# Zaggy1024/RaytracerCore

Hardware: AMD Instinct MI355X
Metric: Mrays/sec (primary+secondary) and samples/sec at 1080p, Cornell box (higher is better)
Workload: dtype f32; 1 GPU; bounce.txt camera 0 1920x1080 x 256 spp per GPU per step; traversal=brute, recursion=10, kernel_build=scene-specialised (hiprtc)

## Files before the change

### include/rtcore.h

```cpp
#ifndef RTCORE_H
#define RTCORE_H

#ifndef __HIPCC_RTC__
#include <stdint.h>
#include <stddef.h>
#endif

#ifdef __cplusplus
extern "C" {
#endif

#define RTCORE_ABI_VERSION 6

typedef enum rt_status {
    RT_OK = 0,
    RT_ERR_ARG = -1,
    RT_ERR_HIP = -2,
    RT_ERR_OOM = -3,
    RT_ERR_NCCL = -4,
    RT_ERR_PARSE = -5,
    RT_ERR_NODEVICE = -6,
    RT_ERR_STATE = -7
} rt_status;

// ... 79 lines not shown
    RT_BVH_BUILDER_GPU = 2
} rt_bvh_builder;

#define RT_BUILD_STATS_COUNT 22

int rt_abi_version(void);
const char* rt_build_info(void);
int rt_device_count(void);
int rt_last_error(char* buf, int32_t cap);

int rt_scene_create(const rt_scene_params* params, const rt_prim* prims, int32_t n_prims,
                    int32_t device, rt_scene** out_scene);
int rt_scene_set_camera(rt_scene* scene, const rt_camera* camera);
int rt_scene_set_traversal(rt_scene* scene, int32_t traversal);
int rt_scene_get_info(const rt_scene* scene, rt_scene_info* info);
void rt_scene_destroy(rt_scene* scene);
int rt_set_bvh_builder(int32_t builder);
int rt_scene_get_build_stats(const rt_scene* scene, double* out, int32_t n);
int rt_set_jit(int32_t on);
int rt_scene_get_jit_error(const rt_scene* scene, char* buf, int32_t cap);
int rt_debug_jit_compile(const char* arch, int32_t grouped, char* log, int32_t cap);
int rt_debug_jit_header(const rt_scene_params* params, const rt_prim* prims, int32_t n_prims, const rt_camera* camera,
                        int32_t grouped, char* buf, int64_t cap);
int rt_scene_check_bvh(rt_scene* scene);
#define RT_LAYOUT_COUNT 10
int rt_debug_brute_layout(const rt_prim* prims, int32_t n_prims, int32_t* out, int32_t n_out);
int rt_debug_item_order(int32_t w, int32_t h, int32_t spp, int32_t chunks, int32_t pool, int32_t band,
                        int32_t band_stride, int32_t band_offset, uint32_t* out, int64_t cap_words, int32_t* info);
int rt_debug_pixels_plan(int32_t kernel, int64_t n, int32_t spp, int32_t* info);
int rt_debug_scene_bound(const rt_prim* prims, int32_t n_prims, float* lo, float* hi, float* info);
int rt_debug_block_cull(const rt_prim* prims, int32_t n_prims, const rt_camera* camera, int32_t width, int32_t height,
                        int32_t x0, int32_t y0, int32_t w, int32_t h, int32_t band, int32_t band_stride,
                        int32_t band_offset, uint8_t* dead, int64_t cap, int32_t* info);
int rt_debug_ray_log(rt_scene* scene, void* d_log, uint32_t cap, void* d_count);
int rt_debug_vn_rehit(const double* v0, const double* e01, const double* e02, int32_t mirror, double u, double v,
                      const float* dir, int32_t* inside, double* t, double* origin);
int rt_debug_trace_rays(rt_scene* scene, const void* d_rays, uint32_t n, void* d_hits, int32_t waves_per_simd,
                        void* d_stats, void* stream, float* ms);

int rt_render_tile(rt_scene* scene, int32_t x0, int32_t y0, int32_t w, int32_t h, int32_t spp,
                   uint64_t seed, uint64_t sample_base, rt_color* sum_rgb, uint32_t* samples,
                   uint32_t* misses, uint64_t* rays_out);

int rt_render_tile_1spp(rt_scene* scene, int32_t x0, int32_t y0, int32_t w, int32_t h,
                        uint64_t seed, uint64_t sample_index, rt_color* out);

int rt_primary_ids(rt_scene* scene, int32_t x0, int32_t y0, int32_t w, int32_t h, int32_t* ids_out);

int rt_bvh_counts(rt_scene* scene, int32_t x0, int32_t y0, int32_t w, int32_t h, int32_t* counts_out);

typedef enum rt_bounce_type {
    RT_BOUNCE_SKIPPED = 0,
    RT_BOUNCE_DIFFUSE = 1,
    RT_BOUNCE_SPECULAR = 2,
    RT_BOUNCE_SPECULAR_FAIL = 3,
    RT_BOUNCE_TRANSMITTED = 4,
    RT_BOUNCE_EMISSION = 5,
    RT_BOUNCE_PURE_BLACK = 6,
    RT_BOUNCE_RECURSION_COMPLETE = 7,
    RT_BOUNCE_MISSED = 8,
    RT_BOUNCE_DEBUG = 9
} rt_bounce_type;

typedef struct rt_debug_ray {
    int32_t prim_id;
    int32_t type;
// ... 167 lines not shown
```

### raytracercore_amd/__init__.py

```python
from __future__ import annotations

import ctypes as C
import enum
import os
from dataclasses import dataclass
from typing import List, Optional, Sequence, Tuple

import numpy as np

_HERE = os.path.dirname(os.path.abspath(__file__))
LIB_PATH = os.path.join(_HERE, "librtcore_hip.so")
REPO_ROOT = os.path.dirname(_HERE)

RT_OK = 0
ABI_VERSION = 6
RT_PRIM_TRIANGLE, RT_PRIM_SPHERE, RT_PRIM_PLANE = 0, 1, 2
RT_FLAG_MIRROR, RT_FLAG_TWOSIDED, RT_FLAG_INVERT, RT_FLAG_HASNORMALS, RT_FLAG_TRANSFORMED = 1, 2, 4, 8, 16
RT_CAMERA_FRUSTUM, RT_CAMERA_ORTHO = 0, 1
RT_TRAVERSAL_AUTO, RT_TRAVERSAL_BRUTE, RT_TRAVERSAL_BVH, RT_TRAVERSAL_BVH2, RT_TRAVERSAL_GROUPED = 0, 1, 2, 3, 4
RT_BVH_BUILDER_AUTO, RT_BVH_BUILDER_HOST, RT_BVH_BUILDER_GPU = 0, 1, 2
(RT_BOUNCE_SKIPPED, RT_BOUNCE_DIFFUSE, RT_BOUNCE_SPECULAR, RT_BOUNCE_SPECULAR_FAIL, RT_BOUNCE_TRANSMITTED,
 RT_BOUNCE_EMISSION, RT_BOUNCE_PURE_BLACK, RT_BOUNCE_RECURSION_COMPLETE, RT_BOUNCE_MISSED, RT_BOUNCE_DEBUG) = range(10)
BOUNCE_TYPE_NAMES = ("Skipped", "Diffuse", "Specular", "SpecularFail", "Transmitted", "Emission", "PureBlack",
                     "RecursionComplete", "Missed", "Debug")
# ... 202 lines not shown
        "rt_scene_set_stats": (C.c_int, [C.c_void_p, C.c_int32]),
        "rt_scene_get_stats": (C.c_int, [C.c_void_p, P(C.c_uint64), C.c_int32]),
        "rt_render_frame_multi": (C.c_int, [P(rt_scene_params), P(rt_prim), C.c_int32, P(rt_camera), C.c_int32,
                                            C.c_int32, C.c_uint64, C.c_uint64, P(rt_color), P(C.c_uint32),
                                            P(C.c_uint32), P(C.c_uint64)]),
        "rt_render_bands": (C.c_int, [C.c_void_p] + [C.c_int32] * 4 + [C.c_uint64, C.c_uint64, P(rt_color),
                                      P(C.c_uint32), P(C.c_uint32), P(C.c_uint64)]),
        "rt_render_bands_device": (C.c_int, [C.c_void_p] + [C.c_int32] * 4 + [C.c_uint64, C.c_uint64] +
                                   [C.c_void_p] * 3 + [C.c_uint64, C.c_void_p, C.c_void_p]),
        "rt_band_rows": (C.c_int, [C.c_int32] * 4),
        "rt_band_slot_rows": (C.c_int, [C.c_int32] * 3),
        "rt_scatter_band_slot": (C.c_int, [C.c_void_p, C.c_uint64] + [C.c_int32] * 5 + [P(rt_color), P(C.c_uint32),
                                                                                       P(C.c_uint32)]),
        "rt_frame_create": (C.c_int, [P(rt_scene_params), P(rt_prim), C.c_int32, P(rt_camera), C.c_int32,
                                      P(C.c_void_p)]),
        "rt_frame_set_camera": (C.c_int, [C.c_void_p, P(rt_camera)]),
        "rt_frame_render": (C.c_int, [C.c_void_p, C.c_int32, C.c_uint64, C.c_uint64, P(rt_color), P(C.c_uint32),
                                      P(C.c_uint32), P(C.c_uint64)]),
        "rt_frame_submit": (C.c_int, [C.c_void_p, C.c_int32, C.c_uint64, C.c_uint64]),
        "rt_frame_collect": (C.c_int, [C.c_void_p, P(rt_color), P(C.c_uint32), P(C.c_uint32), P(C.c_uint64)]),
        "rt_frame_inject_fault": (C.c_int, [C.c_void_p, C.c_int32]),
        "rt_frame_destroy": (None, [C.c_void_p]),
        "rt_parse_scene": (C.c_int, [C.c_char_p, P(rt_scene_params), P(rt_prim), P(C.c_int32), P(rt_camera),
                                     P(C.c_int32)]),
        "rt_sample_output": (C.c_int32, [rt_color, C.c_uint32, C.c_uint32, rt_color, C.c_double, C.c_double]),
        "rt_tonemap_device": (C.c_int, [C.c_void_p, C.c_void_p, C.c_void_p, C.c_int32, C.c_int32, rt_color, C.c_double,
                                        C.c_double, C.c_void_p, C.c_void_p]),
        "rt_ref_bvh_export": (C.c_int, [P(rt_prim), C.c_int32, P(C.c_int32), P(C.c_double), P(C.c_int32),
                                        P(C.c_int32)]),
        "rt_debug_item_order": (C.c_int, [C.c_int32] * 8 + [P(C.c_uint32), C.c_int64, P(C.c_int32)]),
        "rt_debug_scene_bound": (C.c_int, [P(rt_prim), C.c_int32, P(C.c_float), P(C.c_float), P(C.c_float)]),
        "rt_debug_block_cull": (C.c_int, [P(rt_prim), C.c_int32, P(rt_camera)] + [C.c_int32] * 9 +
                                [P(C.c_uint8), C.c_int64, P(C.c_int32)]),
        "rt_debug_ray_log": (C.c_int, [C.c_void_p, C.c_void_p, C.c_uint32, C.c_void_p]),
        "rt_debug_vn_rehit": (C.c_int, [P(C.c_double), P(C.c_double), P(C.c_double), C.c_int32, C.c_double,
                                        C.c_double, P(C.c_float), P(C.c_int32), P(C.c_double), P(C.c_double)]),
        "rt_debug_trace_rays": (C.c_int, [C.c_void_p, C.c_void_p, C.c_uint32, C.c_void_p, C.c_int32, C.c_void_p,
                                          C.c_void_p, P(C.c_float)]),
        "rt_query_rays": (C.c_int, [C.c_void_p, C.c_int32, C.c_void_p, C.c_int64, C.c_void_p]),
        "rt_query_rays_device": (C.c_int, [C.c_void_p, C.c_int32, C.c_void_p, C.c_int64, C.c_void_p, C.c_void_p]),
        "rt_camera_rays": (C.c_int, [P(rt_camera)] + [C.c_int32] * 6 + [C.c_void_p]),
        "rt_select_pixels": (C.c_int, [C.c_void_p, C.c_void_p] + [C.c_int32] * 5 + [C.c_void_p]),
        "rt_select_pixels_device": (C.c_int, [C.c_void_p, C.c_void_p] + [C.c_int32] * 5 + [C.c_void_p, C.c_void_p]),
        "rt_select_rays": (C.c_int, [C.c_void_p, C.c_void_p, C.c_int32, C.c_void_p, C.c_int64, C.c_void_p]),
        "rt_select_rays_device": (C.c_int, [C.c_void_p, C.c_void_p, C.c_int32, C.c_void_p, C.c_int64, C.c_void_p,
                                            C.c_void_p]),
        "rt_debug_select_rays": (C.c_int, [P(rt_prim), C.c_int32, C.c_void_p, C.c_int32, C.c_void_p, C.c_int64,
                                           C.c_void_p]),
        "rt_render_rays": (C.c_int, [C.c_void_p, C.c_void_p, C.c_int64, C.c_int32, C.c_uint64, C.c_uint64, C.c_uint64,
                                     P(rt_color), P(C.c_uint32), P(C.c_uint32), P(C.c_uint64)]),
        "rt_render_rays_device": (C.c_int, [C.c_void_p, C.c_void_p, C.c_int64, C.c_int32, C.c_uint64, C.c_uint64,
                                            C.c_uint64] + [C.c_void_p] * 4 + [C.c_void_p]),
        "rt_occluded_rays": (C.c_int, [C.c_void_p, C.c_int32, C.c_void_p, C.c_void_p, C.c_int64, C.c_void_p]),
        "rt_occluded_rays_device": (C.c_int, [C.c_void_p, C.c_int32, C.c_void_p, C.c_void_p, C.c_int64, C.c_void_p,
                                              C.c_void_p]),
        "rt_render_pixels": (C.c_int, [C.c_void_p, C.c_void_p, C.c_int64, C.c_int32, C.c_uint64, C.c_uint64,
                                       P(rt_color), P(C.c_uint32), P(C.c_uint32), P(C.c_double), P(C.c_uint32),
                                       P(C.c_uint64)]),
        "rt_render_pixels_device": (C.c_int, [C.c_void_p, C.c_void_p, C.c_int64, C.c_int32, C.c_uint64, C.c_uint64] +
                                    [C.c_void_p] * 5 + [C.c_uint64, C.c_void_p, C.c_void_p]),
        "rt_adaptive_select_device": (C.c_int, [P(rt_adaptive_params)] + [C.c_void_p] * 5 + [C.c_uint64, C.c_int32,
                                                C.c_int32, C.c_void_p, C.c_uint32, C.c_void_p, C.c_void_p]),
        "rt_debug_adaptive_select": (C.c_int64, [P(rt_adaptive_params)] + [C.c_void_p] * 5 + [C.c_uint64, C.c_int32,
                                                 C.c_int32, C.c_void_p, C.c_uint32]),
        "rt_debug_pixels_plan": (C.c_int, [C.c_int32, C.c_int64, C.c_int32, P(C.c_int32)]),
        "rt_primary_hits_device": (C.c_int, [C.c_void_p] + [C.c_int32] * 4 + [C.c_void_p, C.c_void_p]),
# ... 102 lines not shown
def scene_bound(prims: Sequence[rt_prim]) -> dict:
    lib = load_library()
    n = len(prims)
    arr = (rt_prim * max(1, n))(*prims)
    lo, hi, info = (C.c_float * 3)(), (C.c_float * 3)(), (C.c_float * 2)()
    state = lib.rt_debug_scene_bound(arr, n, lo, hi, info)
    if state < 0:
        _check(state)
    return {"lo": np.array(lo, np.float32), "hi": np.array(hi, np.float32), "limit": np.float32(info[0]),
            "pad": np.float32(info[1]), "state": int(state)}


def block_cull(prims: Sequence[rt_prim], camera: rt_camera, size: Tuple[int, int],
               window: Optional[Tuple[int, int, int, int]] = None,
               bands: Optional[Tuple[int, int, int]] = None) -> Tuple[np.ndarray, int]:
    lib = load_library()
    n = len(prims)
    arr = (rt_prim * max(1, n))(*prims)
    cam = rt_camera.from_buffer_copy(camera)
    b = bands or (0, 0, 0)
    W, H = size
    rows = lib.rt_band_rows(H, b[0], b[1], b[2]) if bands else H
    x0, y0, w, h = window or (0, 0, W, rows)
    bx, by = (w + 7) // 8, (h + 7) // 8
    dead = np.zeros(max(1, bx * by), np.uint8)
    info = (C.c_int32 * 2)()
    live = lib.rt_debug_block_cull(arr, n, C.byref(cam), W, H, x0, y0, w, h, b[0], b[1], b[2],
                                   dead.ctypes.data_as(C.POINTER(C.c_uint8)), bx * by, info)
    if live < 0:
        _check(live)
    return dead[:bx * by].reshape(by, bx).astype(bool), int(live)


def ref_bvh_export(prims: Sequence[rt_prim]) -> Tuple[np.ndarray, np.ndarray, int, int]:
    lib = load_library()
    n = len(prims)
    arr = (rt_prim * max(1, n))(*prims)
    order = np.zeros(max(1, n), np.int32)
    boxes = np.zeros((max(1, 2 * n), 8), np.float64)
    nodes, depth = C.c_int32(0), C.c_int32(0)
    _check(lib.rt_ref_bvh_export(arr, n, order.ctypes.data_as(C.POINTER(C.c_int32)),
                                 boxes.ctypes.data_as(C.POINTER(C.c_double)), C.byref(nodes), C.byref(depth)))
    return order[:n], boxes[:nodes.value], nodes.value, depth.value


def sample_output(sum_rgb: Tuple[float, float, float], samples: int, misses: int,
                  background=(0.0, 0.0, 0.0), background_alpha: float = 0.0, exposure: float = 1.0) -> int:
    lib = load_library()
    return lib.rt_sample_output(rt_color(*sum_rgb), samples, misses, rt_color(*background), background_alpha, exposure)


def device_count() -> int:
    return load_library().rt_device_count()


def camera_rays(camera: rt_camera, size: Tuple[int, int], x0: int = 0, y0: int = 0, w: Optional[int] = None,
                h: Optional[int] = None) -> np.ndarray:
    lib = load_library()
    if not hasattr(lib, "rt_camera_rays"):
        raise RtError("this build of the library has no rt_camera_rays")
    W, H = int(size[0]), int(size[1])
    w = W - x0 if w is None else w
    h = H - y0 if h is None else h
    out = np.zeros((max(w, 0), max(h, 0)), RAY_DTYPE)
    cam = rt_camera.from_buffer_copy(camera)
    _check(lib.rt_camera_rays(C.byref(cam), W, H, x0, y0, w, h, out.ctypes.data_as(C.c_void_p)))
# ... 627 lines not shown
```

### raytracercore_amd/csrc/api_debug.hip

```cpp
#include <cstdlib>
#include <cstring>

#include "rt_scene.h"

namespace {

int n_bvh_prims(const std::vector<HostPrim>& H)
{
    int nb = 0;
    for (const HostPrim& p : H) nb += p.kind != RT_PRIM_PLANE;
    return nb;
}

HostRecords report_records(const std::vector<HostPrim>& H)
{
    const bool host_tree = builder_for(n_bvh_prims(H)) == RT_BVH_BUILDER_HOST;
    return make_host_records(H, host_tree ? grouping_max_leaf(GroupingTree::LayoutReport, (int)H.size(), false) : 0,
                             group_max_default());
}

}

extern "C" {

// ... 453 lines not shown
                        int32_t band_offset, uint8_t* dead, int64_t cap, int32_t* info)
{
    const bool banded = band > 0;
    if (n_prims < 0 || (n_prims > 0 && !prims) || !camera || width <= 0 || height <= 0 || w <= 0 || h <= 0 || x0 < 0 ||
        y0 < 0 || x0 + w > width || cap < 0 || (cap > 0 && !dead) || band < 0 ||
        (camera->kind != RT_CAMERA_FRUSTUM && camera->kind != RT_CAMERA_ORTHO) ||
        (banded && (band_stride <= 0 || band_offset < 0 || band_offset >= band_stride)) || (!banded && y0 + h > height)) {
        set_error("rt_debug_block_cull: bad argument");
        return RT_ERR_ARG;
    }
    int n_planes = 0;
    for (int i = 0; i < n_prims; i++) {
        if (prims[i].kind < 0 || prims[i].kind > 2) {
            set_error("rt_debug_block_cull: unknown primitive kind at index " + std::to_string(i));
            return RT_ERR_ARG;
        }
        n_planes += prims[i].kind == RT_PRIM_PLANE ? 1 : 0;
    }
    const SceneBound b = make_scene_bound(prepare_prims(prims, n_prims));
    CameraD camd;
    CameraF camf;
    camera_init(*camera, width, height, camd, camf);
    const CullWindow win{x0, y0, w, h, banded ? band : 0, banded ? band_stride : 0, banded ? band_offset : 0};
    std::vector<unsigned char> flags;
    const int live = cull_blocks(camf, b, n_planes, win, flags);
    for (size_t i = 0; i < flags.size() && (int64_t)i < cap; i++) dead[i] = flags[i];
    if (info) {
        info[0] = (w + 7) / 8;
        info[1] = (h + 7) / 8;
    }
    return live;
}

int rt_parse_scene(const char* text, rt_scene_params* params, rt_prim* prims, int32_t* n_prims, rt_camera* cameras,
                   int32_t* n_cameras)
{
    if (!text || !n_prims || !n_cameras) {
        set_error("rt_parse_scene: bad argument");
        return RT_ERR_ARG;
    }
    ParsedScene ps;
    std::string err;
    if (!parse_scene_text(text, ps, err)) {
        set_error(err);
        return RT_ERR_PARSE;
    }
    const int cap_p = *n_prims, cap_c = *n_cameras;
    *n_prims = (int32_t)ps.prims.size();
    *n_cameras = (int32_t)ps.cameras.size();
    if (params) *params = ps.params;
    if (prims) {
        if (cap_p < (int)ps.prims.size()) {
            set_error("rt_parse_scene: primitive array too small");
            return RT_ERR_ARG;
        }
        std::copy(ps.prims.begin(), ps.prims.end(), prims);
    }
    if (cameras) {
        if (cap_c < (int)ps.cameras.size()) {
            set_error("rt_parse_scene: camera array too small");
            return RT_ERR_ARG;
        }
        std::copy(ps.cameras.begin(), ps.cameras.end(), cameras);
    }
    return RT_OK;
}
// ... 27 lines not shown
```

### raytracercore_amd/csrc/kernels_path.hip

```cpp
#include "../../include/rtcore_rng.h"
#include "rt_kernels.h"
#ifdef RT_SCENE_CONST
#include "rt_scene_const.h"
#endif

namespace rtc {
namespace {

struct V3 {
    float x, y, z;
};
__device__ __forceinline__ V3 v3(float x, float y, float z) { return V3{x, y, z}; }
__device__ __forceinline__ V3 xyz(float4 a) { return V3{a.x, a.y, a.z}; }
__device__ __forceinline__ V3 operator+(V3 a, V3 b) { return {a.x + b.x, a.y + b.y, a.z + b.z}; }
__device__ __forceinline__ V3 operator-(V3 a, V3 b) { return {a.x - b.x, a.y - b.y, a.z - b.z}; }
__device__ __forceinline__ V3 operator*(V3 a, float s) { return {a.x * s, a.y * s, a.z * s}; }
__device__ __forceinline__ V3 operator*(V3 a, V3 b) { return {a.x * b.x, a.y * b.y, a.z * b.z}; }
__device__ __forceinline__ V3 operator-(V3 a) { return {-a.x, -a.y, -a.z}; }
__device__ __forceinline__ float dot(V3 a, V3 b) { return fmaf(a.x, b.x, fmaf(a.y, b.y, a.z * b.z)); }
__device__ __forceinline__ bool known_zero(float c)
{
#if defined(RT_SCENE_CONST)
    return __builtin_constant_p(c) && c == 0.0f;
#else
// ... 609 lines not shown
    (void)c;
    return RT_SCENE_CAMERA_KIND == RT_CAMERA_FRUSTUM;
#else
    return c.kind == RT_CAMERA_FRUSTUM;
#endif
}
template <class CamT>
__device__ __forceinline__ bool cam_dof(const CamT& c)
{
#ifdef RT_SCENE_CAMERA_DOF
    (void)c;
    return RT_SCENE_CAMERA_DOF != 0;
#else
    return c.dof != 0.0f;
#endif
}
template <class CamT>
__device__ __forceinline__ Ray3 camera_ray(const CamT& c, float x, float y)
{
    Ray3 r;
    if (cam_frustum(c)) {
        const float ox = fmaf(x, c.tan_x_per_px, -c.tan_x);
        const float oy = fmaf(y, c.tan_y_per_px, -c.tan_y);
        r.d = normalize(madd(xyz(c.up), oy, madd(xyz(c.side), ox, xyz(c.look))));
        r.o = xyz(c.position);
    } else {
        r.o = madd(xyz(c.up), (y - c.h2) * c.v_mult, madd(xyz(c.side), (x - c.w2) * c.h_mult, xyz(c.position)));
        r.d = normalize(xyz(c.look));
    }
    r.o = madd(r.d, c.image_plane, r.o);
    return r;
}

template <bool LEAN = false, class CamT>
__device__ __forceinline__ void start_sample(const CamT& cam, int x, int y, Sample& S)
{
    const float sx = LEAN ? fmaf((float)rt_rng_next24(&S.rng), 0x1p-24f, (float)x) : (float)x + next_u(S.rng);
    const float sy = LEAN ? fmaf((float)rt_rng_next24(&S.rng), 0x1p-24f, (float)y) : (float)y + next_u(S.rng);
    const Ray3 r = camera_ray(cam, sx, sy);
    S.o = r.o;
    S.d = r.d;
    if (cam_dof(cam)) {
        const V3 focus = madd(r.d, cam.focal_length - cam.image_plane, r.o);
        const float dist = fsqrt(next_u(S.rng)) * cam.dof;
        const float turn = next_u(S.rng);
        const float ox = __builtin_amdgcn_cosf(turn) * dist, oy = __builtin_amdgcn_sinf(turn) * dist;
        const Ray3 r2 = camera_ray(cam, sx + ox, sy + oy);
        S.o = r2.o;
        S.d = normalize(focus - r2.o);
    }
    S.tint = v3(1.0f, 1.0f, 1.0f);
    S.bounce = 0;
    S.prev = -1;
}

template <bool LEAN>
__device__ __forceinline__ float one_minus_exp2_2a(float a, float z)
{
    const float x = 2.0f * a * 0.69314718055994531f;
    const float series = -x * fmaf(x, fmaf(x, fmaf(x, 1.0f / 24.0f, 1.0f / 6.0f), 0.5f), 1.0f);
    const float direct = LEAN ? fmaf(-z, z, 1.0f) : 1.0f - __builtin_amdgcn_exp2f(2.0f * a);
    return x > -0.0625f ? series : direct;
}

__host__ __device__ __noinline__ bool vn_rehit_test(const PrimD& P, double u, double v, V3 dir, bool& inside,
                                                   double* t_out = nullptr, double* o_out = nullptr)
{
    const Vec4d a = P.a, e1 = P.b, e2 = P.c;
    const double d[4] = {(double)dir.x, (double)dir.y, (double)dir.z, 0.0};
    const double o[4] = {__builtin_fma(e1.x, u, __builtin_fma(e2.x, v, a.x)), __builtin_fma(e1.y, u, __builtin_fma(e2.y, v, a.y)),
                         __builtin_fma(e1.z, u, __builtin_fma(e2.z, v, a.z)), __builtin_fma(e1.w, u, __builtin_fma(e2.w, v, a.w))};
// ... 342 lines not shown
    QueryRay q;
    q.o = v3((float)r0.x, (float)r0.y, (float)r1.x);
    q.d = v3((float)r2.x, (float)r2.y, (float)r3.x);
    const float inf = __builtin_huge_valf();
    const bool finite = (fabsf(q.o.x) < inf) & (fabsf(q.o.y) < inf) & (fabsf(q.o.z) < inf) & (fabsf(q.d.x) < inf) &
                        (fabsf(q.d.y) < inf) & (fabsf(q.d.z) < inf) & (fabs(r1.y) < __builtin_huge_val()) &
                        (fabs(r3.y) < __builtin_huge_val());
    q.valid = finite & ((q.d.x != 0.0f) | (q.d.y != 0.0f) | (q.d.z != 0.0f));
    return q;
}

template <class ParT>
__device__ __forceinline__ unsigned item_ray(unsigned item, const ParT& p)
{
    return ((item >> (6 + p.log2_chunks)) << 6) | (item & 63u);
}

template <class ParT>
__device__ __forceinline__ void list_pixel(unsigned pix, const ParT& p, int& fx, int& fy)
{
    unsigned q, r;
    divmod(pix, (unsigned)p.scene.width, p.inv_frame_w, q, r);
    fx = (int)r;
    fy = (int)q;
}

template <bool NT, class ParT>
__device__ __forceinline__ int item_sample(const Lane& L, const ParT& p)
{
    if (!NT) return L.s_next;
    const int c = (int)((L.item >> 6) & (unsigned)(p.n_chunks - 1));
    return c * p.chunk + (int)(L.cnt & 0xFFu) + (int)((L.cnt >> 8) & 0xFFu);
}
template <bool NT, int SRC = ITEMS_TILE, class ParT, class SceneT, class CamT>
__device__ __forceinline__ void refill(Lane& L, Sample& S, const ParT& p, const SceneT& s, const CamT& cam, int lane,
                                      unsigned total)
{
    const bool need = L.active && !L.live && (!L.item_open || L.cnt < 65536u);
    if (need && L.item_open) {
        const float4 part = make_float4(L.ar, L.ag, L.ab, __uint_as_float((L.cnt & 0xFFu) | ((L.cnt & 0xFF00u) << 8)));
        if (NT) {
            typedef float nt_f4 __attribute__((ext_vector_type(4)));
            const nt_f4 v = {part.x, part.y, part.z, part.w};
            __builtin_nontemporal_store(v, reinterpret_cast<nt_f4*>(&p.partial[L.item]));
        } else {
            p.partial[L.item] = part;
        }
        L.item_open = false;
        L.ar = L.ag = L.ab = 0.0f;
    }
    const unsigned long long m = __ballot(need);
    if (m) {
        unsigned k = (unsigned)__popcll(m);
        const unsigned avail = L.pool_end - L.pool_next;
        unsigned fresh = 0, fresh_len = (unsigned)p.pool;
        bool draw = k > avail;
        if (!NT && draw && k < (unsigned)p.batch && __ballot(L.active && !need) != 0ull) {
            draw = false;
            k = avail;
        }
        if (draw) {
            const bool linear = p.linear != 0;
            unsigned got = linear ? total : (unsigned)p.n_split << 28;
            if (lane == 0) {
                if (p.n_split <= 1) {
                    const unsigned f = atomicAdd(p.counter, 1u);
                    if (f < p.split_tickets[0]) got = linear ? f * (unsigned)p.pool : f;
// ... 43 lines not shown
                    L.item_open = true;
                    if (!NT) L.s_next = s0;
                    L.cnt = (unsigned)(min(p.spp, s0 + p.chunk) - s0) << 16;
                    if (!NT) {
                        L.fx = (int)ri;
                        L.pkey = rt_rng_pixel_key(p.seed_key, p.stream_base + (unsigned long long)ri);
                    }
                }
            } else {
                int px, py, c, fx, fy;
                item_pixel<!NT>(L.item, p, px, py, c, fx, fy);
                if (px < p.w && py < p.h && c * p.chunk < p.spp) {
                    L.item_open = true;
                    const int s0 = c * p.chunk;
                    if (!NT) L.s_next = s0;
                    L.cnt = (unsigned)(min(p.spp, s0 + p.chunk) - s0) << 16;
                    if (!NT) {
                        L.fx = fx;
                        L.fy = fy;
                    }
                    const unsigned long long pix = (unsigned long long)fy * (unsigned long long)p.scene.width +
                                                   (unsigned long long)fx;
                    if (!NT && p.pkeys) L.pkey = p.pkeys[pix];
                    else if (!NT) L.pkey = rt_rng_pixel_key(p.seed_key, pix);
                }
            }
        }
        if (draw) {
            L.pool_next = fresh + (k - avail);
            L.pool_end = fresh + fresh_len;
        } else {
            L.pool_next += k;
        }
    }
    if constexpr (SRC == ITEMS_RAYS) {
        if (L.active && L.item_open && !L.live && L.cnt >= 65536u) {
            const unsigned ri = NT ? item_ray(L.item, p) : (unsigned)L.fx;
            if (NT) L.pkey = rt_rng_pixel_key(p.seed_key, p.stream_base + (unsigned long long)ri);
            const QueryRay q = load_query_ray(p.ray_list, ri);
            if (q.valid) {
                S.rng = rt_rng_from_pixel_key(L.pkey, p.sample_base + (unsigned long long)item_sample<NT>(L, p));
                (void)rt_rng_next24(&S.rng);
                (void)rt_rng_next24(&S.rng);
                S.o = q.o;
                S.d = q.d;
                S.tint = v3(1.0f, 1.0f, 1.0f);
                S.bounce = 0;
                S.prev = -1;
                L.live = true;
            } else {
                const unsigned left = L.cnt >> 16;
                L.cnt = (L.cnt & 0xFFFFu) + (left << 8);
                if (!NT) L.s_next += (int)left;
            }
        }
        return;
    }
    if (L.active && L.item_open && !L.live && L.cnt >= 65536u) {
        int fx = L.fx, fy = L.fy;
        if (NT && SRC == ITEMS_PIXELS) {
            const unsigned pix = p.pixel_list[item_ray(L.item, p)];
            list_pixel(pix, p, fx, fy);
            L.pkey = rt_rng_pixel_key(p.seed_key, (unsigned long long)pix);
        } else if (NT) {
            int px, py, c;
            item_pixel(L.item, p, px, py, c, fx, fy);
            L.pkey = rt_rng_pixel_key(p.seed_key, (unsigned long long)fy * (unsigned long long)p.scene.width +
                                                      (unsigned long long)fx);
        }
        S.rng = rt_rng_from_pixel_key(L.pkey, p.sample_base + (unsigned long long)item_sample<NT>(L, p));
        start_sample<!NT>(cam, fx, fy, S);
        L.live = true;
    }
}

template <bool VN, bool PIN = false, bool SLOT = false, bool REC = false, class SceneT, class VnP, class TestP, class ParT>
__device__ __forceinline__ void bounce(Lane& L, Sample& S, const SceneT& s, const ShadeRecs& R, VnP vnormals, TestP tests,
                                       const PrimD* prims_d, const Best& b, [[maybe_unused]] const ParT& p)
{
    V3 col;
    [[maybe_unused]] BounceRec rec;
    [[maybe_unused]] const V3 ro = S.o, rd = S.d, rtint = S.tint;
    [[maybe_unused]] const int rbounce = S.bounce;
    [[maybe_unused]] unsigned rsample = 0;
    if constexpr (REC) {
        if (p.rec_rays) {
            int px, py, c, fx, fy;
            item_pixel(L.item, p, px, py, c, fx, fy);
            rsample = ((unsigned)py * (unsigned)p.w + (unsigned)px) * (unsigned)p.spp + (unsigned)item_sample<SLOT>(L, p);
        }
    }
// ... 74 lines not shown
typedef RT_AS_CONST const CameraF CameraC;
typedef RT_AS_CONST const PathParams ParamsC;

template <bool CULL, bool LDS, bool STATS, bool VN, int SRC = ITEMS_TILE>
__device__ __forceinline__ void path_body(const CameraF* __restrict__ camp, const PathParams* __restrict__ pp)
{
    const ParamsC& P0 = *(const ParamsC*)pp;
    extern __shared__ float4 lds_scene[];
    const ShadeRecs R = stage_scene<LDS>(P0.scene, P0.prims, P0.mats, P0.xf, lds_scene);
    const int lane = threadIdx.x & 63;
    const unsigned total = (unsigned)P0.n_chunks * (unsigned)P0.n_pad;
    Lane L;
    lane_init(L);
    Sample S;
    S.prev = -1;
    S.bounce = 0;
    Counters cnt{};
    unsigned long long wave_rays = 0;
    const unsigned long long bound_off = P0.scene_bound != 0 ? 0ull : ~0ull;

    while (true) {
        unsigned long long t0 = 0, t1 = 0, t2 = 0;
        if (STATS) t0 = __builtin_readcyclecounter();
        const CameraC* cp = (const CameraC*)camp;
        asm volatile("" : "+s"(cp));
        const ParamsC* pq = (const ParamsC*)pp;
        asm volatile("" : "+s"(pq));
#ifdef RT_SCENE_CONST
        const PathScene& sc = *(const PathScene*)kSceneW;
#else
        const auto& sc = pq->scene;
#endif
#if defined(RT_SCENE_CONST) && RT_SCENE_CONST_CAMERA
        refill<false>(L, S, *pq, sc, *(const CameraF*)kCameraW, lane, total);
#else
        refill<false, SRC>(L, S, *pq, sc, *cp, lane, total);
#endif
        if (!__any(L.active)) break;
        if (STATS) t1 = __builtin_readcyclecounter();
        wave_rays += (unsigned)__popcll(__ballot(L.live));
        if (L.live) {
#ifdef RT_SCENE_CONST
            const auto tests = (const TestRec*)kTestsW;
            const auto rects = (const RectRec*)kRectsW;
            const auto frames = (const FrameRec*)kFramesW;
            const auto boxes = (const BoxRec*)kFramesW;
            const auto groups = (const GroupRec*)kGroupsW;
            const auto xf = (const XformF*)kXfW;
#else
            const auto tests = (const RT_AS_CONST TestRec*)pq->tests;
            const auto rects = (const RT_AS_CONST RectRec*)pq->rects;
            const auto frames = (const RT_AS_CONST FrameRec*)pq->frames;
            const auto boxes = (const RT_AS_CONST BoxRec*)pq->frames;
            const auto groups = (const RT_AS_CONST GroupRec*)pq->groups;
            const auto xf = (const RT_AS_CONST XformF*)pq->xf;
#endif
            const auto vnormals = (const RT_AS_CONST float4*)pq->vnormals;
            Best b = query_start<VN>(sc, S.prev);
            bool query = true;
            if (!STATS && (!CULL || RT_BOUND_GROUPED) &&
                __builtin_expect((__ballot(L.live && S.bounce != 0) | bound_off) == 0ull, 0))
                query = __any(L.live && scene_meets(sc, S.o, S.d));
            if (query)
                trace_brute<CULL, STATS>(sc, groups, tests, rects, frames, boxes, xf, S.o, S.d, S.prev, b, cnt.tris,
                                         cnt.sphs, cnt.nodes);
            test_planes(sc, tests, S.o, S.d, S.prev, b);
            if (VN && __builtin_isnan(S.d.x + S.d.y + S.d.z)) b = Best{__builtin_huge_valf(), -1};
            if (STATS) t2 = __builtin_readcyclecounter();
            bounce<VN, false, false, STATS>(L, S, sc, R, vnormals, tests, pq->prims_d, b, *pq);
// ... 1239 lines not shown
```

### raytracercore_amd/csrc/launch_params.cpp

```cpp
#include "launch_params.h"

#include <algorithm>
#include <cmath>
#include <cstdlib>

#include "host_scene.h"

namespace rtc {

void set_item_order(PathParams& p)
{
    const char* e = getenv("RTCORE_ITEM_ORDER");
    bool dense = !(e && e[0] == '0');
    const unsigned slots = (unsigned)p.pool / 64u;
    const unsigned used = (unsigned)((p.spp + p.chunk - 1) / p.chunk);
    const unsigned n_blocks = (unsigned)(p.n_pad / 64);
    for (;; dense = false) {
        const unsigned n_real = dense ? used : (unsigned)p.n_chunks;
        const unsigned n_full = dense && p.spp % p.chunk != 0 ? used - 1 : n_real;
        p.tpb = n_full / slots;
        p.tail_first = p.tpb * (unsigned)p.pool;
        p.tail_len = (n_real - p.tpb * slots) * 64u;
        p.magic_tpb = 0;
        if (p.tpb <= 1) break;
// ... 72 lines not shown
    p.spec = 12;
    if (const char* e = getenv("RTCORE_BVH_SPEC")) p.spec = std::max(1, std::min(64, atoi(e)));
    set_blocks(p, p.n_pad / 64);
    p.seed = seed;
    p.seed_key = rt_rng_seed_key(seed);
    p.sample_base = base;
    return p;
}

PathParams make_params_rays(int kernel, int64_t n, int spp, uint64_t seed, uint64_t base, uint64_t stream_base)
{
    PathParams p = make_params_for(kernel, 0, 0, 0, 0, 8, (int)((n + 7) / 8), spp, seed, base, 2073600.0);
    p.n_rays = (unsigned)n;
    p.stream_base = stream_base;
    return p;
}

PathParams make_params_pixels(int kernel, int64_t n, int spp, uint64_t seed, uint64_t base, int width, int height)
{
    PathParams p = make_params_for(kernel, 0, 0, 0, 0, 8, (int)((n + 7) / 8), spp, seed, base, 2073600.0);
    p.n_rays = (unsigned)n;
    p.n_frame_px = (unsigned)((uint64_t)width * (uint64_t)height);
    p.inv_frame_w = 1.0f / (float)width;
    return p;
}

int64_t render_rays_max_n(int kernel, int spp)
{
    const PathParams p = make_params_for(kernel, 0, 0, 0, 0, 8, 8, spp, 0, 0, 2073600.0);
    const int64_t blocks = (int64_t)(0xF0000000ull / ((uint64_t)p.n_chunks * 64u));
    return std::min<int64_t>(blocks * 64, (int64_t)1 << 30);
}

void set_band(PathParams& p, int band, int stride, int offset)
{
    p.band = band;
    p.band_stride = stride;
    p.band_offset = offset;
    p.band_log2 = -1;
    for (int k = 0; k < 31; k++)
        if (band == (1 << k)) p.band_log2 = k;
    p.inv_band = 1.0f / (float)band;
}

int band_set_rows(int H, int band, int stride, int offset)
{
    int rows = 0;
    for (int b = offset; b * band < H; b += stride) rows += std::min(band, H - b * band);
    return rows;
}

int band_slot_rows(int H, int band, int stride)
{
    int m = 0;
    for (int o = 0; o < stride; o++) m = std::max(m, band_set_rows(H, band, stride, o));
    return m;
}

void scatter_band_set(const unsigned char* slot, size_t plane, int W, int H, int band, int stride, int offset,
                      rt_color* sum_rgb, uint32_t* samples, uint32_t* misses)
{
    const double* hs = reinterpret_cast<const double*>(slot);
    const uint32_t* hn = reinterpret_cast<const uint32_t*>(hs + 3 * plane);
    const uint32_t* hm = hn + plane;
    parallel_ranges((size_t)W, 64, [&](size_t xa, size_t xb) {
        int tr = 0;
// ... 31 lines not shown
```

### raytracercore_amd/csrc/launch_params.h

```cpp
#pragma once
#include "rt_kernels.h"

namespace rtc {

PathParams make_params_for(int kernel, int chunks_over, int pool_over, int x0, int y0, int w, int h, int spp,
                           uint64_t seed, uint64_t base, double chunk_npix);
PathParams make_params_rays(int kernel, int64_t n, int spp, uint64_t seed, uint64_t base, uint64_t stream_base);
int64_t render_rays_max_n(int kernel, int spp);
PathParams make_params_pixels(int kernel, int64_t n, int spp, uint64_t seed, uint64_t base, int width, int height);
void set_item_order(PathParams& p);
void set_blocks(PathParams& p, int n_blocks);
void set_band(PathParams& p, int band, int stride, int offset);
int64_t list_tickets(const PathParams& p, uint32_t* out, int64_t cap_words);

int band_set_rows(int H, int band, int stride, int offset);
int band_slot_rows(int H, int band, int stride);
void scatter_band_set(const unsigned char* slot, size_t plane, int W, int H, int band, int stride, int offset,
                      rt_color* sum_rgb, uint32_t* samples, uint32_t* misses);

}
```

### raytracercore_amd/csrc/rt_kernels.h

```cpp
#pragma once
#include "../../include/rtcore_rng.h"
#include "rt_internal.h"

namespace rtc {

constexpr int kMaxSplit = 8;
constexpr int kSplitStride = 32;

enum ItemSource : int { ITEMS_TILE = 0, ITEMS_RAYS = 1, ITEMS_PIXELS = 2 };

struct PathParams {
    int x0, y0, w, h;
    int band, band_stride, band_offset;
    int band_log2;
    float inv_band;
    int spp;
    int chunk;
    int n_chunks;
    int log2_chunks;
    int blocks_x;
    int n_pad;
    int refill;
    int spec;
    int pool;
// ... 10 lines not shown
    unsigned magic_tpb;
    unsigned tail_first;
    unsigned tail_len;
    int linear;
    int batch;
    unsigned split_full[8];
    unsigned split_tickets[8];
    float4* partial;
    unsigned long long* rays;
    int* stack_ovf;
    unsigned long long* stats;
    PathScene scene;
    const TestRec* tests;
    const float4* rows;
    const RectRec* rects;
    const FrameRec* frames;
    const PrimF* prims;
    const GroupRec* groups;
    const NodeF* nodes;
    const Node4Q* nodes4;
    const XformF* xf;
    const MatF* mats;
    const float4* vnormals;
    const PrimD* prims_d;
    float4* ray_log;
    unsigned int* ray_log_n;
    unsigned int ray_log_cap;
    float4* rec_rays;
    float4* rec_samples;
    unsigned int rec_max;
    union {
        const double2* ray_list;
        const uint32_t* pixel_list;
    };
    unsigned int n_rays;
    union {
        unsigned long long stream_base;
        struct {
            unsigned int n_frame_px;
            float inv_frame_w;
        };
    };
    int scene_bound;
    const unsigned int* cull;
};
constexpr int kCullTable = 4;
constexpr int kRecRows = 6;

template <class ParT>
__host__ __device__ inline void ticket_items(const ParT& p, unsigned g, unsigned t, unsigned& first, unsigned& len)
{
    const unsigned full = p.split_full[g];
    unsigned blk, off;
    if (t < full) {
        blk = p.magic_tpb ? (unsigned)(((unsigned long long)t * p.magic_tpb) >> 32) : t;
        off = (t - blk * p.tpb) * (unsigned)p.pool;
        len = (unsigned)p.pool;
    } else {
        blk = t - full;
        off = p.tail_first;
        len = p.tail_len;
    }
    first = p.split_start[g] + (blk << (p.log2_chunks + 6)) + off;
}

struct TraceRaysParams {
    const float4* rays;
    float2* hits;
    unsigned int n;
    unsigned int* counter;
    int* stack_ovf;
    const TestRec* tests;
    const float4* rows;
    const Node4Q* nodes4;
    const XformF* xf;
    int root4;
    int spec;
    const GroupRec* outer;
// ... 95 lines not shown
```

### raytracercore_amd/csrc/rt_scene.h

```cpp
#pragma once
#include <algorithm>
#include <array>
#include <functional>
#include <string>
#include <vector>

#include "block_cull.h"
#include "host_scene.h"
#include "launch_params.h"
#include "rt_jit.h"
#include "rt_kernels.h"
#include "scene_records.h"

using namespace rtc;

#define HIP_TRY(expr)                                                                                  \
    do {                                                                                                \
        hipError_t e_ = (expr);                                                                         \
        if (e_ != hipSuccess) {                                                                         \
            set_error(std::string(#expr) + ": " + hipGetErrorString(e_));                               \
            return e_ == hipErrorOutOfMemory ? RT_ERR_OOM : RT_ERR_HIP;                                 \
        }                                                                                               \
    } while (0)

// ... 98 lines not shown
    struct BruteHost {
        std::vector<GroupRec> groups;
        std::vector<RectRec> rects;
        std::vector<FrameRec> frames;
        std::vector<TestRec> tests;
    } flat_h, grouped_h;
    std::vector<XformF> xf_h;
    unsigned jit_gen = 0;
    struct {
        int variant = -1;
        unsigned gen = 0;
        hipFunction_t fn = nullptr;
        int blocks_per_cu = 0;
        int status = 0;
        double compile_ms = 0;
        bool from_cache = false;
        std::string error;
        std::string header;
    } jit;
    double grouped_measured = 0;
    DevBuf<NodeF> nodes;
    DevBuf<Node4Q> nodes4;
    DevBuf<Node4Q> hot4;
    DevBuf<XformF> xf;
    DevBuf<MatF> mats;
    DevBuf<float4> vnormals;
    DevBuf<PrimD> prims_d;
    DevBuf<XformD> xf_d;
    DevBuf<RefNode> ref_nodes;
    DevBuf<unsigned int> counter;
    DevBuf<rt_key2> pkeys;
    bool pkeys_valid = false;
    uint64_t pkeys_seed = 0;
    DevBuf<int> stack_ovf;
    DevBuf<unsigned long long> rays;
    DevBuf<float4> partial;
    DevBuf<double> sum, colors;
    DevBuf<float> colors32;
    HostBuf<unsigned char> stage;
    HostBuf<unsigned long long> rays_h;
    static constexpr int kCopyChunks = 8;
    std::array<hipEvent_t, kCopyChunks> copy_ev{};
    hipStream_t copy_stream = nullptr;
    std::array<hipEvent_t, kCopyChunks> band_ev{};
    DevBuf<uint32_t> samples, misses;
    DevBuf<int32_t> ids;
    DevBuf<rt_ray> query_rays;
    DevBuf<rt_hit> query_hits;
    std::array<hipEvent_t, 2> query_up_ev{};
    DevBuf<rt_ray> primary_rays;
    DevBuf<double> occluded_t_max;
    DevBuf<unsigned char> occluded_out;
    DevBuf<TileRec> render_rays_recs;
    int rays_variant = -1, rays_blocks_per_cu = 1;
    DevBuf<uint32_t> pixel_list;
    DevBuf<PixelRec> pixel_recs;
    int pixels_variant = -1, pixels_blocks_per_cu = 1;
    DevBuf<rt_select_item> select_items;
    DevBuf<rt_ray> select_rays;
    DevBuf<rt_selection> select_out;
    bool stats_on = false;
    float4* ray_log = nullptr;
    unsigned int* ray_log_n = nullptr;
    unsigned int ray_log_cap = 0;
    int stats_blocks_per_cu = 1;
    DevBuf<unsigned long long> stats_buf;
// ... 93 lines not shown
```

### raytracercore_amd/csrc/scene_upload.hip

```cpp
#include <atomic>
#include <cmath>
#include <cstdio>
#include <cstdlib>
#include <cstring>
#include <unordered_map>

#include "bvh_gpu.h"
#include "rt_scene.h"

namespace rtc {

static std::atomic<int> g_builder{RT_BVH_BUILDER_AUTO};
constexpr int kGpuBuildMin = 1 << 22;

int builder_for(int n_bvh)
{
    int b = g_builder.load();
    if (b == RT_BVH_BUILDER_AUTO)
        if (const char* e = getenv("RTCORE_BVH_BUILDER"))
            b = std::strcmp(e, "gpu") == 0 ? RT_BVH_BUILDER_GPU : std::strcmp(e, "host") == 0 ? RT_BVH_BUILDER_HOST : b;
    if (b == RT_BVH_BUILDER_AUTO) b = n_bvh >= kGpuBuildMin ? RT_BVH_BUILDER_GPU : RT_BVH_BUILDER_HOST;
    return n_bvh > 0 ? b : RT_BVH_BUILDER_HOST;
}

// ... 615 lines not shown
    }
    HIP_TRY(hipMemsetAsync(p.counter, 0, sizeof(unsigned int) * kSplitStride * p.n_split, stream));
    int grid = s->n_cu * (s->stats_on ? s->stats_blocks_per_cu : s->blocks_per_cu);
    p.stack_ovf = nullptr;
    if (s->variant >= 4) {
        HIP_TRY(s->stack_ovf.reserve((size_t)grid * 256 * kStackOverflow));
        p.stack_ovf = s->stack_ovf.p;
    }
    const int jit = s->tracing ? 0 : prepare_jit(s);
    int jit_grid = jit ? s->n_cu * s->jit.blocks_per_cu : 0;
    if ((s->variant >> 1) < 2 && !s->stats_on) {
        constexpr double kSamplesPerLane = 6.0;
        const double samples = ((double)p.w * (double)p.h - (cull ? (double)cull->dead_px : 0.0)) * (double)p.spp;
        int cap = (int)std::ceil(samples / ((double)s->n_cu * 256.0 * kSamplesPerLane));
        if (const char* e = getenv("RTCORE_GRID_BPC")) cap = atoi(e);
        cap = std::max(1, cap);
        if (jit) jit_grid = s->n_cu * std::min(s->jit.blocks_per_cu, cap);
        else grid = s->n_cu * std::min(s->blocks_per_cu, cap);
    }
    const int tslot = (int)(s->launches % rt_scene::kTimeRing);
    if (timed) HIP_TRY(hipEventRecord(s->t_start[tslot], stream));
    fill_launch(s->dev, s->variant, p);
    p.pkeys = nullptr;
    static const bool pkeys_on = !(getenv("RTCORE_PIXEL_KEYS") && getenv("RTCORE_PIXEL_KEYS")[0] == '0');
    if ((s->variant >> 1) < 2 && !s->stats_on && pkeys_on) {
        if (!s->pkeys_valid || s->pkeys_seed != p.seed) {
            HIP_TRY(s->pkeys.reserve((size_t)s->params.width * (size_t)s->params.height));
            HIP_TRY(launch_pixel_keys(p.seed_key, s->params.width, s->params.height, s->pkeys.p, stream));
            s->pkeys_valid = true;
            s->pkeys_seed = p.seed;
        }
        p.pkeys = s->pkeys.p;
    }
    const PathParams* pa = nullptr;
    const int urc = upload_params(s, p, stream, &pa);
    if (urc != RT_OK) return urc;
    if (jit) {
        const CameraF* ca = s->camf_d.p;
        void* args[] = {&ca, &pa};
        HIP_TRY(hipModuleLaunchKernel(s->jit.fn, jit_grid, 1, 1, 256, 1, 1,
                                      (unsigned)path_dyn_lds(s->dev, s->variant), stream, args, nullptr));
    } else {
        HIP_TRY(launch_path(s->dev, s->camf_d.p, pa, s->variant, grid, stream, s->stats_on));
    }
    if (timed) {
        HIP_TRY(hipEventRecord(s->t_end[tslot], stream));
        s->launches++;
    }
    return RT_OK;
}

int end_op(rt_scene* s, hipStream_t stream)
{
    HIP_TRY(hipEventRecord(s->done_ev, stream));
    s->last_stream = stream;
    s->any_op = true;
    return RT_OK;
}

int queue_copy(rt_scene* s, CopyPlan& plan, const void* d_src, size_t a, size_t b, size_t rec_bytes, int k,
               hipStream_t stream)
{
    k = std::max(1, std::min(k, rt_scene::kCopyChunks - plan.n));
    const size_t per = (b - a + k - 1) / k;
    for (int c = 0; c < k; c++) {
        const size_t ca = std::min(b, a + c * per), cb = std::min(b, a + (c + 1) * per);
// ... 62 lines not shown
```

Before: 118,200 Mrays/s.

## Precompute primary camera rays per wave into global start rows at refill

When a wave opens a new work item, it now generates the camera ray directions and RNG state for all samples of that item and writes them to a per-wave global buffer. Later refills for the same item read them back instead of recomputing the pixel sample and camera ray. The aim is to batch the camera-ray setup and cut per-refill arithmetic and divergence. The cost is extra global memory traffic, a scratch buffer of up to 256 MB, and more code paths gated by an environment variable and camera type.

```diff
diff --git a/include/rtcore.h b/include/rtcore.h
--- a/include/rtcore.h
+++ b/include/rtcore.h
@@ -135,6 +135,8 @@
 int rt_debug_block_cull(const rt_prim* prims, int32_t n_prims, const rt_camera* camera, int32_t width, int32_t height,
                         int32_t x0, int32_t y0, int32_t w, int32_t h, int32_t band, int32_t band_stride,
                         int32_t band_offset, uint8_t* dead, int64_t cap, int32_t* info);
+int rt_debug_start_rows(int32_t kernel, const rt_camera* camera, int32_t w, int32_t h, int32_t spp, int32_t chunks,
+                        int32_t grid_blocks, int32_t flags, int64_t* info);
 int rt_debug_ray_log(rt_scene* scene, void* d_log, uint32_t cap, void* d_count);
 int rt_debug_vn_rehit(const double* v0, const double* e01, const double* e02, int32_t mirror, double u, double v,
                       const float* dir, int32_t* inside, double* t, double* origin);
diff --git a/raytracercore_amd/__init__.py b/raytracercore_amd/__init__.py
--- a/raytracercore_amd/__init__.py
+++ b/raytracercore_amd/__init__.py
@@ -258,6 +258,7 @@
         "rt_debug_scene_bound": (C.c_int, [P(rt_prim), C.c_int32, P(C.c_float), P(C.c_float), P(C.c_float)]),
         "rt_debug_block_cull": (C.c_int, [P(rt_prim), C.c_int32, P(rt_camera)] + [C.c_int32] * 9 +
                                 [P(C.c_uint8), C.c_int64, P(C.c_int32)]),
+        "rt_debug_start_rows": (C.c_int, [C.c_int32, P(rt_camera)] + [C.c_int32] * 6 + [P(C.c_int64)]),
         "rt_debug_ray_log": (C.c_int, [C.c_void_p, C.c_void_p, C.c_uint32, C.c_void_p]),
         "rt_debug_vn_rehit": (C.c_int, [P(C.c_double), P(C.c_double), P(C.c_double), C.c_int32, C.c_double,
                                         C.c_double, P(C.c_float), P(C.c_int32), P(C.c_double), P(C.c_double)]),
@@ -426,6 +427,18 @@
     return dead[:bx * by].reshape(by, bx).astype(bool), int(live)
 
 
+def start_rows(kernel: int, camera: rt_camera, w: int, h: int, spp: int, chunks: int = 0, grid_blocks: int = 1792,
+               instrumented: bool = False, vertex_normals: bool = False) -> dict:
+    lib = load_library()
+    cam = rt_camera.from_buffer_copy(camera)
+    info = (C.c_int64 * 3)()
+    on = lib.rt_debug_start_rows(kernel, C.byref(cam), w, h, spp, chunks, grid_blocks,
+                                 int(bool(instrumented)) | int(bool(vertex_normals)) << 1, info)
+    if on < 0:
+        _check(on)
+    return {"on": bool(on), "rows": int(info[0]), "bytes": int(info[1]), "chunk": int(info[2])}
+
+
 def ref_bvh_export(prims: Sequence[rt_prim]) -> Tuple[np.ndarray, np.ndarray, int, int]:
     lib = load_library()
     n = len(prims)
diff --git a/raytracercore_amd/csrc/api_debug.hip b/raytracercore_amd/csrc/api_debug.hip
--- a/raytracercore_amd/csrc/api_debug.hip
+++ b/raytracercore_amd/csrc/api_debug.hip
@@ -509,6 +509,25 @@
     return live;
 }
 
+int rt_debug_start_rows(int32_t kernel, const rt_camera* camera, int32_t w, int32_t h, int32_t spp, int32_t chunks,
+                        int32_t grid_blocks, int32_t flags, int64_t* info)
+{
+    if (kernel < 0 || kernel > 3 || !camera || w <= 0 || h <= 0 || spp <= 0 || chunks < 0 || grid_blocks <= 0 || !info ||
+        (camera->kind != RT_CAMERA_FRUSTUM && camera->kind != RT_CAMERA_ORTHO)) {
+        set_error("rt_debug_start_rows: bad argument");
+        return RT_ERR_ARG;
+    }
+    CameraD camd;
+    CameraF camf;
+    camera_init(*camera, w, h, camd, camf);
+    const PathParams p = make_params_for(kernel, chunks, 0, 0, 0, w, h, spp, 0, 0, 0.0);
+    const StartRowsPlan sr = plan_start_rows(kernel, (flags & 1) != 0, (flags & 2) != 0, camf.kind, camf.dof != 0.0f, p.chunk, grid_blocks);
+    info[0] = sr.rows;
+    info[1] = (int64_t)sr.bytes;
+    info[2] = p.chunk;
+    return sr.on ? 1 : 0;
+}
+
 int rt_parse_scene(const char* text, rt_scene_params* params, rt_prim* prims, int32_t* n_prims, rt_camera* cameras,
                    int32_t* n_cameras)
 {
diff --git a/raytracercore_amd/csrc/kernels_path.hip b/raytracercore_amd/csrc/kernels_path.hip
--- a/raytracercore_amd/csrc/kernels_path.hip
+++ b/raytracercore_amd/csrc/kernels_path.hip
@@ -665,11 +665,17 @@
     return r;
 }
 
+template <bool LEAN>
+__device__ __forceinline__ void sample_point(int x, int y, Sample& S, float& sx, float& sy)
+{
+    sx = LEAN ? fmaf((float)rt_rng_next24(&S.rng), 0x1p-24f, (float)x) : (float)x + next_u(S.rng);
+    sy = LEAN ? fmaf((float)rt_rng_next24(&S.rng), 0x1p-24f, (float)y) : (float)y + next_u(S.rng);
+}
 template <bool LEAN = false, class CamT>
 __device__ __forceinline__ void start_sample(const CamT& cam, int x, int y, Sample& S)
 {
-    const float sx = LEAN ? fmaf((float)rt_rng_next24(&S.rng), 0x1p-24f, (float)x) : (float)x + next_u(S.rng);
-    const float sy = LEAN ? fmaf((float)rt_rng_next24(&S.rng), 0x1p-24f, (float)y) : (float)y + next_u(S.rng);
+    float sx, sy;
+    sample_point<LEAN>(x, y, S, sx, sy);
     const Ray3 r = camera_ray(cam, sx, sy);
     S.o = r.o;
     S.d = r.d;
@@ -1078,7 +1084,34 @@
     const int c = (int)((L.item >> 6) & (unsigned)(p.n_chunks - 1));
     return c * p.chunk + (int)(L.cnt & 0xFFu) + (int)((L.cnt >> 8) & 0xFFu);
 }
-template <bool NT, int SRC = ITEMS_TILE, class ParT, class SceneT, class CamT>
+template <bool NT, int SRC, bool ROWS, class ParT, class CamT>
+__device__ __forceinline__ bool start_rows_on(const ParT& p, [[maybe_unused]] const CamT& cam)
+{
+    if constexpr (NT || SRC != ITEMS_TILE || !ROWS) {
+        return false;
+    } else {
+#ifdef RT_SCENE_CONST
+        if (!cam_frustum(cam) || cam_dof(cam)) return false;
+#endif
+        return p.starts != nullptr;
+    }
+}
+typedef float row_f4 __attribute__((ext_vector_type(4)));
+#ifdef __HIP_DEVICE_COMPILE__
+typedef __attribute__((address_space(1))) row_f4 row_g4;
+typedef __attribute__((address_space(1))) unsigned char row_g1;
+#else
+typedef row_f4 row_g4;
+typedef unsigned char row_g1;
+#endif
+template <class ParT>
+__device__ __forceinline__ unsigned start_row_offset(const ParT& p, unsigned r, int lane)
+{
+    const unsigned wave = blockIdx.x * 4u + (unsigned)__builtin_amdgcn_readfirstlane((int)(threadIdx.x >> 6));
+    return (((wave * (unsigned)p.start_rows + r) << 6) | (unsigned)lane) * 16u;
+}
+
+template <bool NT, int SRC = ITEMS_TILE, bool ROWS = false, class ParT, class SceneT, class CamT>
 __device__ __forceinline__ void refill(Lane& L, Sample& S, const ParT& p, const SceneT& s, const CamT& cam, int lane,
                                       unsigned total)
 {
@@ -1188,6 +1221,20 @@
         } else {
             L.pool_next += k;
         }
+        if (k != 0 && start_rows_on<NT, SRC, ROWS>(p, cam)) {
+            const unsigned n = need && L.item_open ? L.cnt >> 16 : 0u;
+            row_g1* const rows = (row_g1*)(unsigned long long)p.starts;
+            for (unsigned j = 0; j < (unsigned)p.start_rows; j++) {
+                if (j < n) {
+                    S.rng = rt_rng_from_pixel_key(L.pkey, p.sample_base + (unsigned long long)(L.s_next + (int)j));
+                    float sx, sy;
+                    sample_point<true>(L.fx, L.fy, S, sx, sy);
+                    S.d = camera_ray(cam, sx, sy).d;
+                    const row_f4 v = {S.d.x, S.d.y, S.d.z, __uint_as_float(S.rng.x)};
+                    *(row_g4*)(rows + start_row_offset(p, j, lane)) = v;
+                }
+            }
+        }
     }
     if constexpr (SRC == ITEMS_RAYS) {
         if (L.active && L.item_open && !L.live && L.cnt >= 65536u) {
@@ -1213,6 +1260,20 @@
         return;
     }
     if (L.active && L.item_open && !L.live && L.cnt >= 65536u) {
+        if (start_rows_on<NT, SRC, ROWS>(p, cam)) {
+            const unsigned r = (L.cnt & 0xFFu) + ((L.cnt >> 8) & 0xFFu);
+            const row_g1* const rows = (const row_g1*)(unsigned long long)p.starts;
+            const row_f4 v = *(const row_g4*)(rows + start_row_offset(p, r, lane));
+            const V3 d = v3(v.x, v.y, v.z);
+            S.rng.x = __float_as_uint(v.w);
+            S.o = madd(d, cam.image_plane, xyz(cam.position));
+            S.d = d;
+            S.tint = v3(1.0f, 1.0f, 1.0f);
+            S.bounce = 0;
+            S.prev = -1;
+            L.live = true;
+            return;
+        }
         int fx = L.fx, fy = L.fy;
         if (NT && SRC == ITEMS_PIXELS) {
             const unsigned pix = p.pixel_list[item_ray(L.item, p)];
@@ -1353,9 +1414,9 @@
         const auto& sc = pq->scene;
 #endif
 #if defined(RT_SCENE_CONST) && RT_SCENE_CONST_CAMERA
-        refill<false>(L, S, *pq, sc, *(const CameraF*)kCameraW, lane, total);
+        refill<false, ITEMS_TILE, !STATS && !VN>(L, S, *pq, sc, *(const CameraF*)kCameraW, lane, total);
 #else
-        refill<false, SRC>(L, S, *pq, sc, *cp, lane, total);
+        refill<false, SRC, !STATS && !VN>(L, S, *pq, sc, *cp, lane, total);
 #endif
         if (!__any(L.active)) break;
         if (STATS) t1 = __builtin_readcyclecounter();
diff --git a/raytracercore_amd/csrc/launch_params.cpp b/raytracercore_amd/csrc/launch_params.cpp
--- a/raytracercore_amd/csrc/launch_params.cpp
+++ b/raytracercore_amd/csrc/launch_params.cpp
@@ -128,6 +128,19 @@
     return std::min<int64_t>(blocks * 64, (int64_t)1 << 30);
 }
 
+StartRowsPlan plan_start_rows(int kernel, bool instrumented, bool vertex_normals, int camera_kind, bool dof, int chunk,
+                              int grid_blocks)
+{
+    const StartRowsPlan off{false, 0, 0};
+    if (kernel < 0 || kernel >= 2 || instrumented || vertex_normals || camera_kind != RT_CAMERA_FRUSTUM || dof) return off;
+    if (chunk < 1 || chunk > kStartRowsMaxChunk || grid_blocks < 1) return off;
+    if (const char* e = getenv("RTCORE_START_ROWS"))
+        if (atoi(e) == 0) return off;
+    const size_t bytes = (size_t)grid_blocks * 4u * (size_t)chunk * 64u * 16u;
+    if (bytes > kStartRowsCap) return off;
+    return StartRowsPlan{true, chunk, bytes};
+}
+
 void set_band(PathParams& p, int band, int stride, int offset)
 {
     p.band = band;
diff --git a/raytracercore_amd/csrc/launch_params.h b/raytracercore_amd/csrc/launch_params.h
--- a/raytracercore_amd/csrc/launch_params.h
+++ b/raytracercore_amd/csrc/launch_params.h
@@ -13,6 +13,16 @@
 void set_band(PathParams& p, int band, int stride, int offset);
 int64_t list_tickets(const PathParams& p, uint32_t* out, int64_t cap_words);
 
+constexpr int kStartRowsMaxChunk = 16;
+constexpr size_t kStartRowsCap = 256u << 20;
+struct StartRowsPlan {
+    bool on;
+    int rows;
+    size_t bytes;
+};
+StartRowsPlan plan_start_rows(int kernel, bool instrumented, bool vertex_normals, int camera_kind, bool dof, int chunk,
+                              int grid_blocks);
+
 int band_set_rows(int H, int band, int stride, int offset);
 int band_slot_rows(int H, int band, int stride);
 void scatter_band_set(const unsigned char* slot, size_t plane, int W, int H, int band, int stride, int offset,
diff --git a/raytracercore_amd/csrc/rt_kernels.h b/raytracercore_amd/csrc/rt_kernels.h
--- a/raytracercore_amd/csrc/rt_kernels.h
+++ b/raytracercore_amd/csrc/rt_kernels.h
@@ -66,8 +66,10 @@
     union {
         const double2* ray_list;
         const uint32_t* pixel_list;
+        float4* starts;
     };
     unsigned int n_rays;
+    int start_rows;
     union {
         unsigned long long stream_base;
         struct {
@@ -78,6 +80,9 @@
     int scene_bound;
     const unsigned int* cull;
 };
+static_assert(__builtin_offsetof(PathParams, start_rows) == __builtin_offsetof(PathParams, n_rays) + 4 &&
+                  __builtin_offsetof(PathParams, scene_bound) == __builtin_offsetof(PathParams, n_rays) + 16,
+              "start_rows takes the padding after n_rays");
 constexpr int kCullTable = 4;
 constexpr int kRecRows = 6;
 
diff --git a/raytracercore_amd/csrc/rt_scene.h b/raytracercore_amd/csrc/rt_scene.h
--- a/raytracercore_amd/csrc/rt_scene.h
+++ b/raytracercore_amd/csrc/rt_scene.h
@@ -154,6 +154,7 @@
     DevBuf<rt_key2> pkeys;
     bool pkeys_valid = false;
     uint64_t pkeys_seed = 0;
+    DevBuf<float4> starts;
     DevBuf<int> stack_ovf;
     DevBuf<unsigned long long> rays;
     DevBuf<float4> partial;
diff --git a/raytracercore_amd/csrc/scene_upload.hip b/raytracercore_amd/csrc/scene_upload.hip
--- a/raytracercore_amd/csrc/scene_upload.hip
+++ b/raytracercore_amd/csrc/scene_upload.hip
@@ -671,6 +671,15 @@
         }
         p.pkeys = s->pkeys.p;
     }
+    p.starts = nullptr;
+    p.start_rows = 0;
+    const StartRowsPlan sr = plan_start_rows(s->variant >> 1, s->stats_on || s->tracing, s->dev.n_vn > 0, s->camf.kind,
+                                             s->camf.dof != 0.0f, p.chunk, jit ? jit_grid : grid);
+    if (sr.on) {
+        HIP_TRY(s->starts.reserve(sr.bytes / sizeof(float4)));
+        p.starts = s->starts.p;
+        p.start_rows = sr.rows;
+    }
     const PathParams* pa = nullptr;
     const int urc = upload_params(s, p, stream, &pa);
     if (urc != RT_OK) return urc;
```

After: 123,300 Mrays/s, median of 6. 1.04x the previous value.
